# mjq11302010044/TPGSR

Measured on AMD Instinct MI355X. Metric: training img/s (16x64->32x128, bs=48/GPU), TPGSR-TSRN full train step, higher is better.
Workload: dtype bf16x2; 1 GPU; C3: TPGSR-TSRN = TSRN_TL (STN+mask) + CRNN teacher/student text prior, stu_iter 1, full train step (teacher fwd, student fwd+bwd, distill loss, prior dropout, SR fwd+bwd, ImageLoss(gradient), clip 0.25, Adam); tpg=crnn, batch_per_gpu=48, global_batch=48, parallelism=dp1, launch=recorded plans, plain launches: main + weight-gradient + teacher streams

## Files before the change

include/tpgsr_hip.h:

```cpp
#ifndef TPGSR_HIP_H
#define TPGSR_HIP_H

#ifdef __cplusplus
extern "C" {
#endif

#define TPGSR_ACT_NONE 0
#define TPGSR_ACT_RELU 1
#define TPGSR_ACT_MISH 2
#define TPGSR_ACT_TANH 3
#define TPGSR_ACT_PRELU 4

const char* tpgsr_last_error(void);
int tpgsr_version(void);
int tpgsr_sizeof(int which);

typedef struct {
  const float* in;
  const float* in2;
  const float* in_scale;
  const float* in_shift;
  const float* wt;
  const float* bias;
  float* out;
// ... 78 lines not shown
                       int layout, float* dw, float* db, int accumulate, float gscale ,
                       void* stream);

typedef struct tpgsr_wgrad_reduce_desc {
  const float* part;
  const float* dbpart;
  float* dw;
  float* db;
  int Z, K, Cin, Cout, KH, KW, layout, accumulate;
  float gscale;
  int blk0;
  int cin_ld;
  int reserved;
} tpgsr_wgrad_reduce_desc;
int tpgsr_wgrad_reduce_blocks2(int K, int Cin, int Cout, int KH, int KW, int layout, int cin_ld, int has_bias);
int tpgsr_wgrad_reduce_program(const tpgsr_wgrad_reduce_desc* descs_dev, int ndesc, int total_blocks, void* stream);

int tpgsr_pack_conv_weight(const float* w, int Cout, int Cin, int KH, int KW, int transposed, float wscale,
                           float* wt_f, float* wt_d, void* stream);
int tpgsr_pack_tail_weight(const float* w, int Co, int C, int KS, float* wt_f, float* wt_d, void* stream);

typedef struct {
  const float* src;
  float* dst_f;
  float* dst_d;
  int Cout, Cin, KH, KW;
  int kind, f_ld, f_coff;
  float wscale;
  int numel, blk0;
  const float* src2;
  const float* src3;
  int d_ld;
  int cin_ld;
} tpgsr_pack_desc;
typedef struct tpgsr_compose_bwd_desc {
  const float* dWc;
  const float* dbc;
  const float* W1;
  const float* b1;
  const float* wih0;
  const float* wih1;
  float* dW1;
  float* db1;
  float* dwih0;
  float* dwih1;
  float* dbih0;
  float* dbih1;
  int Cin, U, G, blk0;
} tpgsr_compose_bwd_desc;
int tpgsr_compose_bwd_blocks(int Cin, int U, int G);
int tpgsr_compose_bwd_program(const tpgsr_compose_bwd_desc* descs_dev, int ndesc, int total_blocks, void* stream);
int tpgsr_pack_blocks(int kind, int Cout, int Cin, int KH, int KW, long long numel);
int tpgsr_pack_program(const tpgsr_pack_desc* descs_dev, int ndesc, int total_blocks, void* stream);
typedef struct tpgsr_split_desc {
  const float* src;
  void* dst;
  int K, N, ld, kp, blk0;
  int cin;
} tpgsr_split_desc;
int tpgsr_split_bf_blocks(int K, int N);
int tpgsr_split_bf_program(const tpgsr_split_desc* descs_dev, int ndesc, int total_blocks, void* stream);
int tpgsr_bicubic_resize(const float* in_nchw, int N, int Ctot, int C, int H, int W, int OH, int OW, float scale, float shift,
                         float* out_nhwc, void* stream);
int tpgsr_aster_attention(const float* xproj, const float* sproj, const float* wv, const float* bv, const float* x, int N, int T, int A,
                          int D, float* alpha, float* context, void* stream);
int tpgsr_embed_concat(const int* ids, const float* emb, int V, int E, const float* ctx, int D, int N, float* out, void* stream);
int tpgsr_gru_cell(const float* gi, const float* gh, const float* h, int N, int Hd, float* hnew, void* stream);
int tpgsr_softmax_max(const float* logits, int N, int C, int* ids, float* score, int ld, int col, int* ids_next, void* stream);

void tpgsr_halo3_set_enabled(int on);
void tpgsr_wgrad3_set_enabled(int on);
void tpgsr_halo_set_colmajor_min_bytes(long long v);
void tpgsr_halo_set_min_taps(int v);
void tpgsr_halo_set_ne9(int on);
void tpgsr_panel_set_enabled(int on);
void tpgsr_panel_set_min_m(long long m);
void tpgsr_panel_set_k192(int on);
int tpgsr_halo_capacity(const tpgsr_conv_args* a);
int tpgsr_halo_trace(unsigned long long* buf);
int tpgsr_tr_probe(int* out, void* stream);
int tpgsr_mfma_bf16_probe(const void* a, const void* b, const float* c, float* d, int reps, void* stream);
int tpgsr_mfma_probe(float* out, int blocks, int iters, void* stream);
int tpgsr_copy(const float* src, float* dst, long long n, void* stream);
int tpgsr_zero(float* dst, long long n, void* stream);

// ... 230 lines not shown
```

tpgsr_amd/_lib.py:

```python
import ctypes as C
import os

import torch

_HERE = os.path.dirname(os.path.abspath(__file__))
LIB_PATH = os.path.join(_HERE, "libtpgsr_hip.so")

ACT_NONE, ACT_RELU, ACT_MISH, ACT_TANH, ACT_PRELU = 0, 1, 2, 3, 4
_ACT = {None: 0, "none": 0, "relu": 1, "mish": 2, "tanh": 3}

vp = C.c_void_p
ci = C.c_int
ll = C.c_longlong
cf = C.c_float


class ConvArgs(C.Structure):
    _fields_ = [("in_", vp), ("in2", vp), ("in_scale", vp), ("in_shift", vp), ("wt", vp), ("bias", vp), ("out", vp),
                ("bn_partial", vp),
                ("N", ci), ("H", ci), ("W", ci), ("Cin", ci),
                ("in_ld", ci), ("in_coff", ci), ("in2_ld", ci), ("in_act", ci), ("in_ps", ci),
                ("Cout", ci), ("KH", ci), ("KW", ci), ("pad_h", ci), ("pad_w", ci), ("OH", ci), ("OW", ci),
                ("out_ld", ci), ("out_coff", ci), ("out_act", ci), ("out_ps", ci),
                ("in_b", vp), ("cin_a", ci), ("in_b_ld", ci), ("in_dil_w", ci), ("wt_ld", ci), ("wt_coff", ci), ("stride_w", ci),
                ("terms", ci), ("kp", ci), ("wt_bf", vp), ("wt_bf_cin", ci), ("reserved0", ci),
                ("bnb_y", vp), ("bnb_mean", vp), ("bnb_rstd", vp), ("bnb_scale", vp), ("bnb_shift", vp), ("bnb_act", ci), ("bnb_store_dz", ci),
                ("fin_mode", ci), ("fin_accumulate", ci), ("fin_count", ll), ("fin_counter", vp), ("fin_gamma", vp), ("fin_beta", vp),
                ("fin_bias", vp), ("fin_scale", vp), ("fin_shift", vp), ("fin_mean", vp), ("fin_rstd", vp), ("fin_rm", vp), ("fin_rv", vp),
                ("fin_momentum", cf), ("fin_eps", cf), ("bn_row_tiles", ci), ("reserved1", ci), ("in2_scale", vp),
                ("sk_part", vp), ("sk_splits", ci), ("reserved2", ci)]


class WgradArgs(C.Structure):
    _fields_ = [("c", ConvArgs), ("dy", vp), ("dy_ld", ci), ("dy_coff", ci), ("dy_ps", ci), ("part", vp), ("dbpart", vp),
                ("zsplits", ci), ("reserved1", ci), ("dy_bf", vp)]


class GruWgradArgs(C.Structure):
    _fields_ = [("c", ConvArgs), ("dgi", vp), ("dghn", vp), ("h", vp), ("partC", vp), ("dbC", vp), ("partH", vp), ("dbH", vp),
                ("axis", ci), ("zsplits", ci)]


class BigruProjArgs(C.Structure):
    _fields_ = [("c", ConvArgs), ("w_hh", vp), ("b_hh", vp), ("h_out", vp), ("gates", vp), ("axis", ci), ("reserved", ci)]


class PackDesc(C.Structure):
    _fields_ = [("src", vp), ("dst_f", vp), ("dst_d", vp), ("Cout", ci), ("Cin", ci), ("KH", ci), ("KW", ci),
                ("kind", ci), ("f_ld", ci), ("f_coff", ci), ("wscale", cf), ("numel", ci), ("blk0", ci),
                ("src2", vp), ("src3", vp), ("d_ld", ci), ("cin_ld", ci)]


class ComposeBwdDesc(C.Structure):
    _fields_ = [("dWc", vp), ("dbc", vp), ("W1", vp), ("b1", vp), ("wih0", vp), ("wih1", vp), ("dW1", vp), ("db1", vp),
                ("dwih0", vp), ("dwih1", vp), ("dbih0", vp), ("dbih1", vp), ("Cin", ci), ("U", ci), ("G", ci), ("blk0", ci)]


class WgradReduceDesc(C.Structure):
    _fields_ = [("part", vp), ("dbpart", vp), ("dw", vp), ("db", vp), ("Z", ci), ("K", ci), ("Cin", ci), ("Cout", ci),
                ("KH", ci), ("KW", ci), ("layout", ci), ("accumulate", ci), ("gscale", cf), ("blk0", ci), ("cin_ld", ci),
                ("reserved", ci)]


class SplitDesc(C.Structure):
    _fields_ = [("src", vp), ("dst", vp), ("K", ci), ("N", ci), ("ld", ci), ("kp", ci), ("blk0", ci), ("cin", ci)]


class WgradBatchItem(C.Structure):
    _fields_ = [("w", WgradArgs), ("M", ci), ("K", ci), ("MB", ci), ("blk0", ci), ("nblk", ci), ("reserved0", ci), ("reserved1", ci), ("reserved2", ci)]


class ImageDesc(C.Structure):
    _fields_ = [("offset", ll), ("H", ci), ("W", ci), ("xb_off", ci), ("xk_off", ci), ("kx", ci), ("yb_off", ci), ("yk_off", ci), ("ky", ci)]


class BnDerive(C.Structure):
    _fields_ = [("rows", vp), ("nrows", ci), ("C", ci), ("count", ll), ("bias", vp), ("gamma", vp), ("beta", vp),
                ("running_mean", vp), ("running_var", vp), ("momentum", cf), ("eps", cf), ("scale", vp), ("shift", vp),
                ("save_mean", vp), ("save_rstd", vp), ("dgamma", vp), ("dbeta", vp), ("coef", vp), ("accumulate", ci), ("reserved", ci), ("flag", vp)]


class PlanArg(C.Union):
    _fields_ = [("p", vp), ("i", ll), ("f", C.c_double)]
# ... 7 lines not shown
    "tpgsr_plan_add_fork": (ci, [vp]),
    "tpgsr_plan_add_join": (ci, [vp]),
    "tpgsr_plan_set_arg": (ci, [vp, ci, ci, C.POINTER(PlanArg)]),
    "tpgsr_plan_run": (ci, [vp, vp, vp]),
    "tpgsr_plan_add_edge": (ci, [vp, ci, ci]),
    "tpgsr_plan_run3": (ci, [vp, vp, vp, vp]),
    "tpgsr_stream_create": (vp, [C.POINTER(C.c_uint), ci]),
    "tpgsr_plan_set_mode": (None, [ci, ci, C.c_ulonglong, ci]),
    "tpgsr_plan_get_mode": (ci, []),
    "tpgsr_plan_fuzz_point": (ci, [vp]),
    "tpgsr_spin": (ci, [ci, ci, cf, ci, vp]),
    "tpgsr_plan_set_stamp": (ci, [ci]),
    "tpgsr_plan_stamp_epoch": (ci, [vp]),
    "tpgsr_plan_read_stamps": (ci, [vp, C.POINTER(cf), C.POINTER(C.c_longlong), ci]),
    "tpgsr_stream_destroy": (ci, [vp]),
    "tpgsr_pack_program": (ci, [vp, ci, ci, vp]),
    "tpgsr_mfma_probe": (ci, [vp, ci, ci, vp]),
    "tpgsr_copy": (ci, [vp, vp, ll, vp]),
    "tpgsr_zero": (ci, [vp, ll, vp]),
    "tpgsr_version": (ci, []),
    "tpgsr_sizeof": (ci, [ci]),
    "tpgsr_conv_fwd": (ci, [C.POINTER(ConvArgs), vp]),
    "tpgsr_bigru_proj_supported": (ci, [C.POINTER(BigruProjArgs)]),
    "tpgsr_bigru_proj_fwd": (ci, [C.POINTER(BigruProjArgs), vp]),
    "tpgsr_bigru_proj_set_enabled": (None, [ci]),
    "tpgsr_affine_act_bnd": (ci, [C.POINTER(BnDerive), vp, ll, ci, vp, vp]),
    "tpgsr_affine_act_pool_bnd": (ci, [C.POINTER(BnDerive), vp, ci, ci, ci, ci, ci, ci, vp, vp]),
    "tpgsr_bn_bwd_apply_bnd": (ci, [C.POINTER(BnDerive), vp, vp, vp, ll, vp, vp, ci, vp, vp]),
    "tpgsr_wgrad_splits": (ci, [ci, ci, ci]),
    "tpgsr_conv_wgrad": (ci, [C.POINTER(WgradArgs), vp]),
    "tpgsr_wgrad_halo_plan": (ci, [C.POINTER(ConvArgs), C.POINTER(ci), C.POINTER(C.c_longlong)]),
    "tpgsr_wgrad_reduce": (ci, [vp, vp, ci, ci, ci, ci, ci, ci, ci, vp, vp, ci, cf, vp]),
    "tpgsr_pack_blocks": (ci, [ci, ci, ci, ci, ci, ll]),
    "tpgsr_conv_wgrad_batch_prepare": (ci, [C.POINTER(WgradArgs), C.POINTER(WgradBatchItem)]),
    "tpgsr_conv_wgrad_batch": (ci, [vp, ci, ci, ci, ci, vp]),
    "tpgsr_wgrad_reduce_blocks2": (ci, [ci, ci, ci, ci, ci, ci, ci, ci]),
    "tpgsr_wgrad_reduce_program": (ci, [vp, ci, ci, vp]),
    "tpgsr_compose_bwd_blocks": (ci, [ci, ci, ci]),
    "tpgsr_compose_bwd_program": (ci, [vp, ci, ci, vp]),
    "tpgsr_pack_conv_weight": (ci, [vp, ci, ci, ci, ci, ci, cf, vp, vp, vp]),
    "tpgsr_pack_tail_weight": (ci, [vp, ci, ci, ci, vp, vp, vp]),
    "tpgsr_bn_finalize": (ci, [vp, ci, ci, ll, vp, vp, vp, vp, vp, cf, cf, ci, vp, vp, vp, vp, vp]),
    "tpgsr_bn_stats": (ci, [vp, ll, ci, ci, vp, ci, vp]),
    "tpgsr_bn_bwd_reduce": (ci, [vp, vp, vp, ll, ci, vp, vp, vp, vp, ci, vp, ci, vp]),
    "tpgsr_bn_bwd_finalize": (ci, [vp, ci, ci, ll, vp, vp, vp, vp, vp, ci, vp, vp]),
    "tpgsr_bn_bwd_apply": (ci, [vp, vp, vp, ll, ci, vp, vp, ci, vp, vp, vp]),
    "tpgsr_affine_act": (ci, [vp, ll, ci, vp, vp, ci, vp, vp]),
    "tpgsr_affine_act_pool": (ci, [vp, ci, ci, ci, ci, vp, vp, ci, ci, ci, vp, vp]),
    "tpgsr_affine_act_pool_bwd": (ci, [vp, vp, ci, ci, ci, ci, vp, vp, ci, ci, ci, vp, vp]),
    "tpgsr_prelu_fwd": (ci, [vp, vp, ll, vp, vp]),
    "tpgsr_prelu_bwd": (ci, [vp, vp, vp, vp, ll, vp, vp, ci, vp]),
    "tpgsr_add": (ci, [vp, vp, ll, vp, vp]),
    "tpgsr_act_bwd": (ci, [vp, vp, ll, ci, vp, vp]),
    "tpgsr_nchw_to_nhwc": (ci, [vp, ci, ci, ci, ci, vp, vp]),
    "tpgsr_nhwc_to_nchw": (ci, [vp, ci, ci, ci, ci, vp, vp]),
    "tpgsr_reduce_partials": (ci, [vp, ci, ci, vp, ci, vp]),
    "tpgsr_bigru_fwd": (ci, [vp, vp, vp, ci, ci, ci, ci, vp, vp, vp]),
    "tpgsr_bigru_bwd": (ci, [vp, vp, vp, vp, vp, ci, ci, ci, ci, vp, vp, vp]),
    "tpgsr_bigru_bwd2": (ci, [vp, vp, vp, vp, vp, ci, ci, ci, ci, vp, vp, vp]),
    "tpgsr_gru_gate_math_probe": (ci, [vp, vp, vp, ci, vp]),
    "tpgsr_gru_wgrad_splits": (ci, [ll]),
    "tpgsr_gru_wgrad": (ci, [C.POINTER(GruWgradArgs), vp]),
    "tpgsr_tps_grid_fwd": (ci, [vp, vp, vp, ci, ci, ci, vp, vp, vp]),
    "tpgsr_tps_grid_bwd": (ci, [vp, vp, vp, vp, ci, ci, ci, vp, vp]),
    "tpgsr_grid_sample_fwd": (ci, [vp, vp, ci, ci, ci, ci, ci, ci, ci, vp, vp]),
    "tpgsr_grid_sample_bwd": (ci, [vp, vp, vp, ci, ci, ci, ci, ci, ci, ci, vp, vp, vp]),
# ... 127 lines not shown
```

tpgsr_amd/csrc/conv_mfma.hip:

```cpp
#include "common.h"
#include <stdlib.h>
#include <mutex>

#ifndef TPGSR_FRAG_PRELOAD
#define TPGSR_FRAG_PRELOAD 0
#endif
#include "conv_loader.h"

template <int LD, int SPLIT>
__global__ __launch_bounds__(256 * SPLIT) void conv_fwd_kernel(tpgsr_conv_args a, int M, int K, int vecB) {
  constexpr bool VEC_A = LD >= 0;
  __shared__ float As_[SPLIT][KC][ALD];
  __shared__ float Bs_[SPLIT][KC][BN];
  const int grp = SPLIT > 1 ? (int)(threadIdx.x >> 8) : 0;
  float (*As)[ALD] = As_[grp];
  float (*Bs)[BN] = Bs_[grp];
  const int tid = threadIdx.x & 255;
  const int lane = tid & 63, wave = tid >> 6;
  const int wm = wave & 1, wn = wave >> 1;
  const int nbn = (a.Cout + BN - 1) / BN;
  const int tile = xcd_remap(blockIdx.x, gridDim.x);
  const int mblk = tile / nbn;
  const int m0 = mblk * BM, n0 = (tile - mblk * nbn) * BN;
  const int nchunks_all = (K + KC - 1) / KC;
  const int nchunks = (nchunks_all + SPLIT - 1) / SPLIT;
  const int ch0 = grp * nchunks;

  const int aq = tid & 7;
  const int am0 = tid >> 3;
  PixelPos px0 = decode_pixel(a, m0 + am0, M);
  PixelPos px1 = decode_pixel(a, m0 + am0 + 32, M);
  const int bk0 = tid >> 4;
  const int bc = (tid & 15) * 4;

  float4 ra0, ra1, rb0, rb1;
  ARaw qa0, qa1;
  float4 qs = make_float4(1.f, 1.f, 1.f, 1.f), qt = make_float4(0.f, 0.f, 0.f, 0.f);
  constexpr int LDV = LD < 0 ? 0 : LD;
  const int Wr_ = real_w(a);
  const size_t in_floats = a.in_ps ? (size_t)a.N * a.H * a.W * a.Cin : (size_t)a.N * a.H * Wr_ * a.in_ld;
// ... 847 lines not shown
  if (idx >= total) return;
  int kw = idx % KS;
  size_t r = idx / KS;
  int kh = r % KS;
  r /= KS;
  int ci = r % C;
  int co = (int)(r / C);
  float v = w[idx];
  int NP = KS * Co;
  int np = kw * Co + co;
  if (wt_f) wt_f[((size_t)kh * C + ci) * NP + np] = v;
  if (wt_d) wt_d[((size_t)(KS - 1 - kh) * NP + np) * C + ci] = v;
}

extern "C" int tpgsr_pack_tail_weight(const float* w, int Co, int C, int KS, float* wt_f, float* wt_d, void* stream) {
  TPGSR_CHECK_ARG(w && (wt_f || wt_d), "tpgsr_pack_tail_weight: null pointer");
  size_t total = (size_t)Co * C * KS * KS;
  hipLaunchKernelGGL(pack_tail_weight_kernel, dim3(cdiv(total, 256)), dim3(256), 0, (hipStream_t)stream, w, Co, C, KS,
                     wt_f, wt_d);
  TPGSR_LAUNCH_CHECK("tpgsr_pack_tail_weight");
}

#define PK_TILED_MAX_TAPS 9
__host__ __device__ __forceinline__ bool pack_tiled(int kind, int Cout, int Cin, int KH, int KW) {
  return kind == 0 && KH * KW <= PK_TILED_MAX_TAPS && (long long)Cout * Cin >= 65536;
}
__host__ __device__ __forceinline__ int pack_desc_blocks(int kind, int Cout, int Cin, int KH, int KW, long long numel) {
  if (pack_tiled(kind, Cout, Cin, KH, KW)) return ((Cout + 31) / 32) * ((Cin + 31) / 32);
  return (int)((numel + 255) / 256);
}
extern "C" int tpgsr_pack_blocks(int kind, int Cout, int Cin, int KH, int KW, long long numel) {
  return pack_desc_blocks(kind, Cout, Cin, KH, KW, numel);
}

__global__ __launch_bounds__(256) void pack_program_kernel(const tpgsr_pack_desc* __restrict__ descs, int ndesc) {
  __shared__ int s_d;
  __shared__ float tile[32 * (32 * PK_TILED_MAX_TAPS + 1)];
  if (threadIdx.x == 0) {
    int lo = 0, hi = ndesc - 1;
    while (lo < hi) {
      int mid = (lo + hi + 1) >> 1;
      if (descs[mid].blk0 <= (int)blockIdx.x) lo = mid; else hi = mid - 1;
    }
    s_d = lo;
  }
  __syncthreads();
  const tpgsr_pack_desc d = descs[s_d];
  if (pack_tiled(d.kind, d.Cout, d.Cin, d.KH, d.KW)) {
    const int taps = d.KH * d.KW, R = 32 * taps, pitch = R | 1;
    const int nci = (d.Cin + 31) / 32;
    const int b = (int)blockIdx.x - d.blk0;
    const int co0 = (b / nci) * 32, ci0 = (b - (b / nci) * nci) * 32;
    const int cw = min(32, d.Cin - ci0) * taps;
    for (int e = threadIdx.x; e < 32 * R; e += 256) {
      const int row = e / R, pos = e - row * R;
      float v = 0.f;
      if (co0 + row < d.Cout && pos < cw) v = d.src[((size_t)(co0 + row) * d.Cin + ci0) * taps + pos] * d.wscale;
      tile[row * pitch + pos] = v;
    }
    __syncthreads();
    const int cin_ld = d.cin_ld > 0 ? d.cin_ld : d.Cin, d_ld = d.d_ld > 0 ? d.d_ld : d.Cin;
    if (d.dst_f) {
      for (int e = threadIdx.x; e < 32 * R; e += 256) {
        const int co_l = e & 31, rest = e >> 5;
        const int ci_l = rest & 31, tap = rest >> 5;
        if (co0 + co_l < d.Cout && ci0 + ci_l < d.Cin)
          d.dst_f[((size_t)tap * cin_ld + ci0 + ci_l) * d.f_ld + d.f_coff + co0 + co_l] = tile[co_l * pitch + ci_l * taps + tap];
      }
    }
    if (d.dst_d) {
      for (int e = threadIdx.x; e < 32 * R; e += 256) {
        const int ci_l = e & 31, rest = e >> 5;
        const int co_l = rest & 31, tap = rest >> 5;
        const int kh = tap / d.KW, kw = tap - kh * d.KW;
        if (co0 + co_l < d.Cout && ci0 + ci_l < d.Cin)
          d.dst_d[((size_t)((d.KH - 1 - kh) * d.KW + (d.KW - 1 - kw)) * d.Cout + co0 + co_l) * d_ld + ci0 + ci_l] = tile[co_l * pitch + ci_l * taps + tap];
      }
    }
    return;
  }
  long long idx = (long long)(blockIdx.x - d.blk0) * 256 + threadIdx.x;
  if (idx >= d.numel) return;
  if (d.kind == 5) {
    const int U = d.KH;
    const int g = (int)(idx / d.Cin), ci = (int)(idx - (long long)g * d.Cin);
    const float* wr = d.src + (size_t)g * U;
    float a0 = 0.f, a1 = 0.f, a2 = 0.f, a3 = 0.f;
    for (int u = 0; u < U; u += 4) {
      a0 = fmaf(wr[u], d.src2[(size_t)u * d.Cin + ci], a0);
      a1 = fmaf(wr[u + 1], d.src2[(size_t)(u + 1) * d.Cin + ci], a1);
      a2 = fmaf(wr[u + 2], d.src2[(size_t)(u + 2) * d.Cin + ci], a2);
      a3 = fmaf(wr[u + 3], d.src2[(size_t)(u + 3) * d.Cin + ci], a3);
    }
    const float v = (a0 + a1) + (a2 + a3);
    if (d.dst_f) d.dst_f[(size_t)ci * d.f_ld + d.f_coff + g] = v;
    if (d.dst_d) d.dst_d[(size_t)(d.f_coff + g) * d.Cin + ci] = v;
    return;
  }
  if (d.kind == 6) {
    const int U = d.KH, g = (int)idx;
    const float* wr = d.src + (size_t)g * U;
    float a0 = 0.f, a1 = 0.f;
    for (int u = 0; u < U; u += 2) {
      a0 = fmaf(wr[u], d.src2[u], a0);
      a1 = fmaf(wr[u + 1], d.src2[u + 1], a1);
    }
    d.dst_f[d.f_coff + g] = (a0 + a1) + d.src3[g];
    return;
  }
  float v = d.src[idx] * d.wscale;
  if (d.kind == 2) {
// ... 159 lines not shown
```

tpgsr_amd/engine.py:

```python
from __future__ import annotations

import contextlib
import ctypes as C
import math
import os
from typing import Dict, List, Optional

import torch

from . import kernels as K
from ._lib import PackDesc
from .kernels import ConvGeom, Plan, recording

F32 = torch.float32


class ParamArena:

    def __init__(self, module: torch.nn.Module):
        self.module = module
        self.flat: Optional[torch.Tensor] = None
        self.grad: Optional[torch.Tensor] = None
        self.offsets: Dict[str, int] = {}
        self.numel = 0
# ... 488 lines not shown
        from ._lib import ComposeBwdDesc, load
        lib = load()
        arr = (ComposeBwdDesc * len(items))()
        blk, keep = 0, []
        for d, (L, dWc, dbc) in zip(arr, items):
            P, G, gp = self.P, self.G, L.gp
            t = dict(dWc=dWc, dbc=dbc, W1=P[L.w1name], b1=P[L.b1name], wih0=P[gp + "weight_ih_l0"], wih1=P[gp + "weight_ih_l0_reverse"],
                     dW1=G[L.w1name], db1=G[L.b1name], dwih0=G[gp + "weight_ih_l0"], dwih1=G[gp + "weight_ih_l0_reverse"],
                     dbih0=G[gp + "bias_ih_l0"], dbih1=G[gp + "bias_ih_l0_reverse"])
            for k, v in t.items():
                setattr(d, k, v.data_ptr())
            keep += list(t.values())
            d.Cin, d.U, d.G, d.blk0 = L.Cin, L.U, 96, blk
            blk += lib.tpgsr_compose_bwd_blocks(L.Cin, L.U, 96)
        table = torch.frombuffer(bytearray(bytes(arr)), dtype=torch.uint8).to(self.device)
        if K._REC is not None:
            K._REC.keep += keep
        with K.side():
            K.compose_bwd_program(table, len(items), blk)

    def add_pack(self, src, dst_f, dst_d, Cout=0, Cin=0, KH=1, KW=1, kind=0, f_ld=0, f_coff=0, wscale=1.0, src2=None, src3=None,
                 numel=None, d_ld=0, cin_ld=0):
        self._pack.append((src, dst_f, dst_d, Cout, Cin, KH, KW, kind, f_ld, f_coff, wscale, src2, src3, numel, d_ld, cin_ld,
                           getattr(self, "_pack_group", 0)))

    def register_operand(self, *tensors, cins=None):
        for i, t in enumerate(tensors):
            if t is not None:
                assert t.dim() == 2 and t.is_contiguous()
                self._operands.append(t)
                t._tpgsr_cin = K.block_order_cin(t.shape[0], cins[i] if cins else 0)
                t._tpgsr_group = getattr(self, "_pack_group", 0)

    def _finish_split_table(self):
        from ._lib import SplitDesc, load
        self._split_tabs = {}
        self._split_n = 0
        ops, seen = [], set()
        for t in self._operands:
            if t.data_ptr() not in seen:
                seen.add(t.data_ptr())
                ops.append(t)
        if K.POLICY == "f32" or not ops:
            return
        lib = load()
        self._split_keep = []
        for grp in sorted({getattr(t, "_tpgsr_group", 0) for t in ops}):
            sel = [t for t in ops if getattr(t, "_tpgsr_group", 0) == grp]
            arr = (SplitDesc * len(sel))()
            blk = 0
            for d, t in zip(arr, sel):
                Kd, N = t.shape
                kp = (Kd + 31) // 32 * 32
                twin = torch.zeros(3 * ((N + 31) // 32 * 32) * kp, dtype=torch.bfloat16, device=self.device)
                cin = getattr(t, "_tpgsr_cin", 0)
                K.register_bf_twin(t, twin, kp, cin)
                d.src, d.dst, d.K, d.N, d.ld, d.kp, d.blk0, d.cin = t.data_ptr(), twin.data_ptr(), Kd, N, N, kp, blk, cin
                blk += lib.tpgsr_split_bf_blocks(Kd, N)
                self._split_keep += [t, twin]
            self._split_tabs[grp] = (torch.frombuffer(bytearray(bytes(arr)), dtype=torch.uint8).to(self.device), len(sel), blk)
        self._split_n = len(ops)

    def _finish_pack_table(self):
        from ._lib import load
        lib = load()
        self._pack_tabs = {}
        self._pack_keep = []
        for grp in sorted({e[16] for e in self._pack}):
            sel = [e for e in self._pack if e[16] == grp]
            arr = (PackDesc * len(sel))()
            blk = 0
            for d, (src, dst_f, dst_d, Cout, Cin, KH, KW, kind, f_ld, f_coff, wscale, src2, src3, numel, d_ld, cin_ld, _g) in zip(arr, sel):
                d.src, d.dst_f = src.data_ptr(), dst_f.data_ptr()
                d.dst_d = dst_d.data_ptr() if dst_d is not None else None
                d.src2 = src2.data_ptr() if src2 is not None else None
                d.src3 = src3.data_ptr() if src3 is not None else None
                d.Cout, d.Cin, d.KH, d.KW, d.kind, d.f_ld, d.f_coff, d.wscale = Cout, Cin, KH, KW, kind, f_ld, f_coff, wscale
                d.d_ld, d.cin_ld = d_ld, cin_ld
                cnt = src.numel() if numel is None else numel
                d.numel, d.blk0 = cnt, blk
                blk += lib.tpgsr_pack_blocks(kind, Cout, Cin, KH, KW, cnt)
                self._pack_keep += [src, dst_f, dst_d, src2, src3]
            self._pack_tabs[grp] = (torch.frombuffer(bytearray(bytes(arr)), dtype=torch.uint8).to(self.device), len(sel), blk)

    def pack_group(self, grp):
        if grp in self._pack_tabs:
            K.pack_program(*self._pack_tabs[grp])
        if grp in self._split_tabs:
            K.split_bf_program(*self._split_tabs[grp])

    def pack_all(self):
        for grp in sorted(set(self._pack_tabs) | set(self._split_tabs)):
            self.pack_group(grp)

    def _param_key(self):
        return (sum(p._version for p in self.P.values()), self._kernel_writes, self.arena.flat.data_ptr(), bool(getattr(self, "_split_tabs", None)))

    @staticmethod
    def _plan_splits(plan) -> bool:
        v = getattr(plan, "_tpgsr_splits", None)
        if v is None:
            v = any(op[0] == "tpgsr_split_bf_program" for op in plan.ops)
            try:
                plan._tpgsr_splits = v
            except AttributeError:
                pass
        return v

    def pack_if_stale(self, pack_plan):
        capturing = (not K.DRYRUN) and torch.cuda.is_current_stream_capturing()
        key = self._param_key()
        check = (not K.DRYRUN) and (not capturing) and os.environ.get("TPGSR_PACK_CHECK") == "1"
        splits = self._plan_splits(pack_plan)
        if capturing or key != self._packed_key or (splits and not self._packed_split) or os.environ.get("TPGSR_PACK_ALWAYS") == "1":
            pack_plan.run()
            self._packed_key = None if capturing else key
            self._packed_split = splits
            if check:
                self._packed_sum = self._arena_checksum()
        elif check and getattr(self, "_packed_sum", None) is not None and self._arena_checksum() != self._packed_sum:
            raise RuntimeError(f"{type(self.module).__name__}: the parameters changed behind torch's version counters since the operands were "
                               "packed (a write through p.data / a raw pointer / a flat arena view?) -- call module._engine().invalidate_packed() "
                               "after such writes (TPGSR_PACK_CHECK=1 found this)")

    def _arena_checksum(self):
        w = self.arena.flat.view(torch.int32).to(torch.int64)
        return (int(w.sum().item()), int((w * w).sum().item()))

    def invalidate_packed(self):
        self._kernel_writes += 1
        self._packed_key = None

    def note_packed(self):
        self._packed_key = self._param_key()
        self._packed_split = bool(K.CONV_TERMS)

    def bind(self, device):
        rebuilt = self.arena.ensure(device)
        if not rebuilt and self.device == device:
            return
        self.device = device
        self._plans.clear()
        self._packed_key = None
        self._scratch.clear()
        self._live.clear()
        self._pack = []
        self._operands = []
        self._bn_layers = []
        m = self.module
        self.P = dict(m.named_parameters())
        self.B = dict(m.named_buffers())
        self.G = {}
        for name, p in self.P.items():
            o = self.arena.offsets[name]
            self.G[name] = self.arena.grad[o:o + p.numel()]
        for name, b in self.B.items():
            if b.device != device:
                raise RuntimeError(f"buffer {name} is on {b.device}, parameters on {device}: call module.to(device) first")
        self._build_layers()
        self._finish_pack_table()
        self._finish_split_table()

    def flush_counters(self):
        if self._pending_batches and self.device is not None:
            for n, b in self.B.items():
                if n.endswith("num_batches_tracked"):
                    b += self._pending_batches
        self._pending_batches = 0

    def _two_pass(self, key, record):
        if key not in self._plans:
            if K.POLICY != "f32" and self._operands and not self._split_tabs:
                self._finish_split_table()
            ws = _Ws(self.device)
            record(ws, False)
            self._plans[key] = record(ws, True)
        return self._plans[key]


class TSRNEngine(_EngineBase):

    STN_POOLS = [(2, 2), (2, 2), (2, 2), (2, 2), (1, 2), (1, 1)]

    def __init__(self, module: torch.nn.Module, grid_align_corners: bool = False):
        super().__init__(module)
        self.grid_align_corners = grid_align_corners
        self.overlap_wgrad = os.environ.get("TPGSR_OVERLAP_WGRAD", "1") != "0"
        self.defer_reduce = os.environ.get("TPGSR_DEFER_REDUCE", "1") != "0"
        self.leaf_stn = os.environ.get("TPGSR_LEAF_STN", "1") != "0"
        self.leaf_early = os.environ.get("TPGSR_LEAF_EARLY", "0") == "1"
        self.leaf_strip = os.environ.get("TPGSR_LEAF_STRIP", "1") != "0"
        self.split_leaf_reduce = os.environ.get("TPGSR_SPLIT_LEAF_REDUCE", "1") != "0"
        self.side_batch_blocks = max(1, int(os.environ.get("TPGSR_SIDE_BATCH_BLOCKS", "2")))
        self.side_batch_tail = os.environ.get("TPGSR_SIDE_BATCH_TAIL", "1") != "0"

    def _build_layers(self):
        m = self.module
        self.in_planes = m.in_planes
        self.srb = m.srb_nums
        self.stn = bool(m.stn)
        self.C = self.P["block1.0.weight"].shape[0]
        self.block1 = ConvLayer(self, "block1.0.weight", "block1.0.bias", 9, 9, 4, 4, need_dgrad=False)
        self.block1_dx = FoldedDgrad(self, "block1.0.weight") if self.stn else None
        self.tl = hasattr(m, "infoGen")
        self.rrb = []
        for i in range(self.srb):
# ... 442 lines not shown
```

tpgsr_amd/engine_crnn.py:

```python
from __future__ import annotations

import os
from typing import Optional

import torch

from . import kernels as K
from .engine import BNLayer, ConvLayer, F32, _EngineBase
from .kernels import ConvGeom, Plan, recording


class Conv0Im2col:

    def __init__(self, eng, wname, bname):
        self.eng, self.wname, self.bname = eng, wname, bname
        self.w, self.b = eng.P[wname], eng.P[bname]
        assert tuple(self.w.shape[1:]) == (1, 3, 3)
        self.Cout, self.Cin = self.w.shape[0], 12
        dev = eng.device
        self.wt_f = torch.zeros(12, self.Cout, dtype=F32, device=dev)
        self.wt_d = torch.zeros(self.Cout, 12, dtype=F32, device=dev)
        eng.add_pack(self.w, self.wt_f, self.wt_d, Cout=self.Cout, Cin=9, KH=1, KW=1, kind=0, f_ld=self.Cout, d_ld=12)
        eng.register_operand(self.wt_f, self.wt_d)

# ... 35 lines not shown

    def wgrad(self, N, H, W, x, dy_p):
        eng, g = self.eng, ConvGeom(N, H, W, self.Cin, self.Cout)
        Z = K.wgrad_splits(g.M, g.K, g.Cout)
        part, dbp = eng.wgrad_buffers(Z * g.K * g.Cout, Z * g.Cout)
        with K.side():
            K.conv_wgrad(K.make_wgrad_args(K.make_conv_args(g, x), dy_p, part, dbp, dy_ld=self.Cp))
            K.wgrad_reduce(part, dbp, Z, g, eng.G[self.wname], eng.G[self.bname], accumulate=True)


class LstmLayer:

    def __init__(self, eng, prefix: str):
        self.eng, self.prefix = eng, prefix
        P, dev = eng.P, eng.device
        r = prefix + ".rnn."
        self.r = r
        self.Hh = Hh = P[r + "weight_hh_l0"].shape[1]
        self.Cin = Cin = P[r + "weight_ih_l0"].shape[1]
        G4 = 4 * Hh
        self.wih_f = torch.empty(Cin, 2 * G4, dtype=F32, device=dev)
        self.wih_d = torch.empty(2 * G4, Cin, dtype=F32, device=dev)
        self.bih = torch.empty(2 * G4, dtype=F32, device=dev)
        self.bhh = torch.empty(2, G4, dtype=F32, device=dev)
        self.whh_f = torch.empty(2, Hh, G4, dtype=F32, device=dev)
        for d, suf in enumerate(("", "_reverse")):
            eng.add_pack(P[r + "weight_ih_l0" + suf], self.wih_f, self.wih_d[d * G4:(d + 1) * G4], Cout=G4, Cin=Cin, kind=0,
                         f_ld=2 * G4, f_coff=d * G4)
            eng.add_pack(P[r + "bias_ih_l0" + suf], self.bih[d * G4:(d + 1) * G4], None, kind=2)
            eng.add_pack(P[r + "bias_hh_l0" + suf], self.bhh[d], None, kind=2)
            eng.add_pack(P[r + "weight_hh_l0" + suf], self.whh_f[d], None, Cout=G4, Cin=Hh, kind=0, f_ld=G4)
        eng.register_operand(self.wih_f, self.wih_d)
        nout = P[prefix + ".embedding.weight"].shape[0]
        self.emb = (ConvLayer if nout % 4 == 0 else PaddedLinear)(eng, prefix + ".embedding.weight", prefix + ".embedding.bias")

    def fwd(self, N, T, x, G, gh, Cst, out, e, **loader):
        Hh, G4, P = self.Hh, 4 * self.Hh, self.eng.P
        K.conv_fwd(K.make_conv_args(ConvGeom(N, 1, T, self.Cin, 2 * G4), x, self.wih_f, G, bias=self.bih, **loader))
        if K.LSTM_SEQ and Hh == 256 and N <= 64 and K.lstm_seq_coresident(self.eng.device):
            if not hasattr(self, "_seq"):
                self._seq = {}
            gran = K.LSTM_GRANULE and T <= 31
            key = (K.current_stream().cuda_stream, gran, N)
            if key not in self._seq:
                self._seq[key] = K.lstm_seq_granule_buffers(self.eng.device) if gran else K.lstm_seq_buffers(self.eng.device)
            hx, sync = self._seq[key]
            (K.lstm_seq_fwdg if gran else K.lstm_seq_fwd)(G, self.whh_f, self.bhh, Cst, out, hx, sync, N, T, Hh)
            self.emb.fwd(N, 1, T, out, e)
            return
        S = Hh // (32 * K.LSTM_FWD_KCHUNKS)
        for s in range(T):
            if s > 0:
                a = [out.data_ptr() + 4 * ((s - 1 if d == 0 else T - s) * 2 * Hh + d * Hh) for d in range(2)]
                K.lstm_rec_gemm(a[0], a[1], T * 2 * Hh, self.whh_f[0], self.whh_f[1], N, Hh, G4, S, gh)
            K.lstm_step_fwd(G, gh if s > 0 else None, S, self.bhh, Cst, out, N, T, Hh, s)
        self.emb.fwd(N, 1, T, out, e)

    def bwd(self, N, T, x, G, Cst, out, de, dout, dhc, dcc, dx, dx_bnb=None, **loader):
        eng, P, Gd, r = self.eng, self.eng.P, self.eng.G, self.r
        Hh, G4 = self.Hh, 4 * self.Hh
        batch = K.LSTM_WGRAD_BATCH and K.CONV_TERMS > 0 and K.deferring() and isinstance(self.emb, (ConvLayer, PaddedLinear))
        if not batch:
            self.emb.wgrad(N, 1, T, out, de)
        self.emb.dgrad(N, 1, T, de, dout)
        S = G4 // (32 * K.LSTM_BWD_KCHUNKS)
        seq = K.LSTM_SEQ_BWD and Hh == 256 and N <= 64 and K.lstm_seq_coresident(self.eng.device)
        if seq:
# ... 300 lines not shown
```

Before: 8821 img/s.

## Fuse bf16 triple-split twin writes into the tiled weight pack kernel

The tiled weight-pack kernel now also writes the three-way bf16 split twins (MFMA tiled layout) directly from its shared-memory tile, for operands whose every pack entry qualifies. Those operands are dropped from the separate split_bf program. This removes a per-step read and rewrite of packed f32 weights. The cost is more complex descriptor planning and eligibility checks, with a risk of layout mismatch on edge cases. The CRNN PaddedLinear embedding is also forced into pack group 0.

```diff
diff --git a/include/tpgsr_hip.h b/include/tpgsr_hip.h
--- a/include/tpgsr_hip.h
+++ b/include/tpgsr_hip.h
@@ -134,6 +134,10 @@
   const float* src3;
   int d_ld;
   int cin_ld;
+  void* bf_f;
+  void* bf_d;
+  int bf_f_kp, bf_f_nb32, bf_f_cin, bf_f_koff;
+  int bf_d_kp, bf_d_nb32, bf_d_cin, bf_d_koff;
 } tpgsr_pack_desc;
 typedef struct tpgsr_compose_bwd_desc {
   const float* dWc;
@@ -153,6 +157,7 @@
 int tpgsr_compose_bwd_blocks(int Cin, int U, int G);
 int tpgsr_compose_bwd_program(const tpgsr_compose_bwd_desc* descs_dev, int ndesc, int total_blocks, void* stream);
 int tpgsr_pack_blocks(int kind, int Cout, int Cin, int KH, int KW, long long numel);
+int tpgsr_pack_tiled(int kind, int Cout, int Cin, int KH, int KW);
 int tpgsr_pack_program(const tpgsr_pack_desc* descs_dev, int ndesc, int total_blocks, void* stream);
 typedef struct tpgsr_split_desc {
   const float* src;
diff --git a/tpgsr_amd/_lib.py b/tpgsr_amd/_lib.py
--- a/tpgsr_amd/_lib.py
+++ b/tpgsr_amd/_lib.py
@@ -48,7 +48,9 @@
 class PackDesc(C.Structure):
     _fields_ = [("src", vp), ("dst_f", vp), ("dst_d", vp), ("Cout", ci), ("Cin", ci), ("KH", ci), ("KW", ci),
                 ("kind", ci), ("f_ld", ci), ("f_coff", ci), ("wscale", cf), ("numel", ci), ("blk0", ci),
-                ("src2", vp), ("src3", vp), ("d_ld", ci), ("cin_ld", ci)]
+                ("src2", vp), ("src3", vp), ("d_ld", ci), ("cin_ld", ci), ("bf_f", vp), ("bf_d", vp),
+                ("bf_f_kp", ci), ("bf_f_nb32", ci), ("bf_f_cin", ci), ("bf_f_koff", ci),
+                ("bf_d_kp", ci), ("bf_d_nb32", ci), ("bf_d_cin", ci), ("bf_d_koff", ci)]
 
 
 class ComposeBwdDesc(C.Structure):
@@ -122,6 +124,7 @@
     "tpgsr_wgrad_halo_plan": (ci, [C.POINTER(ConvArgs), C.POINTER(ci), C.POINTER(C.c_longlong)]),
     "tpgsr_wgrad_reduce": (ci, [vp, vp, ci, ci, ci, ci, ci, ci, ci, vp, vp, ci, cf, vp]),
     "tpgsr_pack_blocks": (ci, [ci, ci, ci, ci, ci, ll]),
+    "tpgsr_pack_tiled": (ci, [ci, ci, ci, ci, ci]),
     "tpgsr_conv_wgrad_batch_prepare": (ci, [C.POINTER(WgradArgs), C.POINTER(WgradBatchItem)]),
     "tpgsr_conv_wgrad_batch": (ci, [vp, ci, ci, ci, ci, vp]),
     "tpgsr_wgrad_reduce_blocks2": (ci, [ci, ci, ci, ci, ci, ci, ci, ci]),
diff --git a/tpgsr_amd/csrc/conv_mfma.hip b/tpgsr_amd/csrc/conv_mfma.hip
--- a/tpgsr_amd/csrc/conv_mfma.hip
+++ b/tpgsr_amd/csrc/conv_mfma.hip
@@ -6,6 +6,7 @@
 #define TPGSR_FRAG_PRELOAD 0
 #endif
 #include "conv_loader.h"
+#include "conv_xbf_common.h"
 
 template <int LD, int SPLIT>
 __global__ __launch_bounds__(256 * SPLIT) void conv_fwd_kernel(tpgsr_conv_args a, int M, int K, int vecB) {
@@ -919,6 +920,7 @@
 extern "C" int tpgsr_pack_blocks(int kind, int Cout, int Cin, int KH, int KW, long long numel) {
   return pack_desc_blocks(kind, Cout, Cin, KH, KW, numel);
 }
+extern "C" int tpgsr_pack_tiled(int kind, int Cout, int Cin, int KH, int KW) { return pack_tiled(kind, Cout, Cin, KH, KW) ? 1 : 0; }
 
 __global__ __launch_bounds__(256) void pack_program_kernel(const tpgsr_pack_desc* __restrict__ descs, int ndesc) {
   __shared__ int s_d;
@@ -964,6 +966,54 @@
           d.dst_d[((size_t)((d.KH - 1 - kh) * d.KW + (d.KW - 1 - kw)) * d.Cout + co0 + co_l) * d_ld + ci0 + ci_l] = tile[co_l * pitch + ci_l * taps + tap];
       }
     }
+    if (d.bf_f) {
+      const int KB16 = d.bf_f_kp >> 4;
+      const size_t plane = (size_t)d.bf_f_nb32 * KB16 * 512;
+      unsigned short* dst = reinterpret_cast<unsigned short*>(d.bf_f);
+      for (int e = threadIdx.x; e < 128 * taps; e += 256) {
+        const int co_l = e & 31, g = (e >> 5) & 3, tap = e >> 7;
+        const int cig = ci0 + g * 8;
+        const int k = d.bf_f_cin > 0 ? ((ci0 >> 5) * taps + tap) * 32 + g * 8 : d.bf_f_koff + tap * cin_ld + cig;
+        if (co0 + co_l >= d.Cout || cig >= cin_ld || k >= d.bf_f_kp) continue;
+        __bf16 h[8][3];
+#pragma unroll
+        for (int j = 0; j < 8; ++j) split_bf<3>(tile[co_l * pitch + (g * 8 + j) * taps + tap], h[j]);
+        const int nn = d.f_coff + co0 + co_l;
+        const size_t off = ((((size_t)(nn >> 5) * KB16 + (k >> 4)) * 64) + ((k >> 3) & 1) * 32 + (nn & 31)) * 8;
+#pragma unroll
+        for (int t = 0; t < 3; ++t) {
+          bf16x8 v;
+#pragma unroll
+          for (int j = 0; j < 8; ++j) v[j] = h[j][t];
+          *reinterpret_cast<bf16x8*>(dst + t * plane + off) = v;
+        }
+      }
+    }
+    if (d.bf_d) {
+      const int KB16 = d.bf_d_kp >> 4;
+      const size_t plane = (size_t)d.bf_d_nb32 * KB16 * 512;
+      unsigned short* dst = reinterpret_cast<unsigned short*>(d.bf_d);
+      for (int e = threadIdx.x; e < 128 * taps; e += 256) {
+        const int ci_l = e & 31, g = (e >> 5) & 3, tap = e >> 7;
+        const int kh = tap / d.KW, kw = tap - kh * d.KW;
+        const int tf = (d.KH - 1 - kh) * d.KW + (d.KW - 1 - kw);
+        const int cog = co0 + g * 8;
+        const int k = d.bf_d_cin > 0 ? ((co0 >> 5) * taps + tf) * 32 + g * 8 : d.bf_d_koff + tf * d.Cout + cog;
+        if (ci0 + ci_l >= d.Cin || cog >= d.Cout || k >= d.bf_d_kp) continue;
+        __bf16 h[8][3];
+#pragma unroll
+        for (int j = 0; j < 8; ++j) split_bf<3>(tile[(g * 8 + j) * pitch + ci_l * taps + tap], h[j]);
+        const int nn = ci0 + ci_l;
+        const size_t off = ((((size_t)(nn >> 5) * KB16 + (k >> 4)) * 64) + ((k >> 3) & 1) * 32 + (nn & 31)) * 8;
+#pragma unroll
+        for (int t = 0; t < 3; ++t) {
+          bf16x8 v;
+#pragma unroll
+          for (int j = 0; j < 8; ++j) v[j] = h[j][t];
+          *reinterpret_cast<bf16x8*>(dst + t * plane + off) = v;
+        }
+      }
+    }
     return;
   }
   long long idx = (long long)(blockIdx.x - d.blk0) * 256 + threadIdx.x;
diff --git a/tpgsr_amd/engine.py b/tpgsr_amd/engine.py
--- a/tpgsr_amd/engine.py
+++ b/tpgsr_amd/engine.py
@@ -544,69 +544,130 @@
                 t._tpgsr_cin = K.block_order_cin(t.shape[0], cins[i] if cins else 0)
                 t._tpgsr_group = getattr(self, "_pack_group", 0)
 
+    def _make_twins(self):
+        self._twins = False
+        self._split_ops, seen = [], set()
+        for t in self._operands:
+            if t.data_ptr() not in seen:
+                seen.add(t.data_ptr())
+                self._split_ops.append(t)
+        if K.POLICY == "f32" or not self._split_ops:
+            return
+        self._split_keep = []
+        for t in self._split_ops:
+            Kd, N = t.shape
+            kp = (Kd + 31) // 32 * 32
+            twin = torch.zeros(3 * ((N + 31) // 32 * 32) * kp, dtype=torch.bfloat16, device=self.device)
+            K.register_bf_twin(t, twin, kp, getattr(t, "_tpgsr_cin", 0))
+            self._split_keep += [t, twin]
+        self._twins = True
+
+    def _plane_target(self, e, lib):
+        src, dst_f, dst_d, Cout, Cin, KH, KW, kind, f_ld, f_coff, wscale, src2, src3, numel, d_ld, cin_ld, _g = e
+        tiled = self._twins and bool(lib.tpgsr_pack_tiled(kind, Cout, Cin, KH, KW))
+        taps, out = KH * KW, []
+        for side, dst in (("f", dst_f), ("d", dst_d)):
+            if dst is None:
+                continue
+            hit = None
+            for t in self._split_ops:
+                o = dst.data_ptr() - t.data_ptr()
+                if 0 <= o < t.numel() * 4:
+                    hit = (t,) + divmod(o // 4, t.shape[1])
+                    break
+            if hit is None:
+                continue
+            t, row, col = hit
+            tw, fields = getattr(t, "_tpgsr_twin", None), None
+            if tiled and tw is not None and col == 0:
+                kp, cin_t = tw[1], tw[2]
+                ch, ld, own = (cin_ld or Cin, f_ld, Cin) if side == "f" else (Cout, d_ld or Cin, Cout)
+                ok = ld == t.shape[1] and (f_coff % 32 == 0 if side == "f" else True)
+                if cin_t > 0:
+                    ok = ok and cin_t == own == ch and row == 0 and t.shape[0] == taps * ch
+                else:
+                    ok = ok and ch % 8 == 0 and row % 8 == 0
+                if ok:
+                    fields = (tw[0], kp, (t.shape[1] + 31) // 32, cin_t, row)
+            out.append((side, t, fields))
+        return out
+
+    def _finish_pack_table(self):
+        from ._lib import load
+        lib = load()
+        self._pack_tabs = {}
+        self._pack_keep = []
+        self._pack_planes = set()
+        targets = [self._plane_target(e, lib) for e in self._pack]
+        whole = {}
+        for tg in targets:
+            for side, t, fields in tg:
+                whole[t.data_ptr()] = whole.get(t.data_ptr(), True) and fields is not None
+        self._plane_ops = {p for p, ok in whole.items() if ok}
+        for grp in sorted({e[16] for e in self._pack}):
+            sel = [(e, tg) for e, tg in zip(self._pack, targets) if e[16] == grp]
+            arr = (PackDesc * len(sel))()
+            blk = 0
+            for d, ((src, dst_f, dst_d, Cout, Cin, KH, KW, kind, f_ld, f_coff, wscale, src2, src3, numel, d_ld, cin_ld, _g), tg) in zip(arr, sel):
+                d.src, d.dst_f = src.data_ptr(), dst_f.data_ptr()
+                d.dst_d = dst_d.data_ptr() if dst_d is not None else None
+                d.src2 = src2.data_ptr() if src2 is not None else None
+                d.src3 = src3.data_ptr() if src3 is not None else None
+                d.Cout, d.Cin, d.KH, d.KW, d.kind, d.f_ld, d.f_coff, d.wscale = Cout, Cin, KH, KW, kind, f_ld, f_coff, wscale
+                d.d_ld, d.cin_ld = d_ld, cin_ld
+                for side, t, fields in tg:
+                    if t.data_ptr() in self._plane_ops:
+                        twin, kp, nb32, cin_t, row = fields
+                        if side == "f":
+                            d.bf_f, d.bf_f_kp, d.bf_f_nb32, d.bf_f_cin, d.bf_f_koff = twin.data_ptr(), kp, nb32, cin_t, row
+                        else:
+                            d.bf_d, d.bf_d_kp, d.bf_d_nb32, d.bf_d_cin, d.bf_d_koff = twin.data_ptr(), kp, nb32, cin_t, row
+                        self._pack_planes.add(grp)
+                cnt = src.numel() if numel is None else numel
+                d.numel, d.blk0 = cnt, blk
+                blk += lib.tpgsr_pack_blocks(kind, Cout, Cin, KH, KW, cnt)
+                self._pack_keep += [src, dst_f, dst_d, src2, src3]
+            self._pack_tabs[grp] = (torch.frombuffer(bytearray(bytes(arr)), dtype=torch.uint8).to(self.device), len(sel), blk)
+
     def _finish_split_table(self):
         from ._lib import SplitDesc, load
         self._split_tabs = {}
         self._split_n = 0
-        ops, seen = [], set()
-        for t in self._operands:
-            if t.data_ptr() not in seen:
-                seen.add(t.data_ptr())
-                ops.append(t)
-        if K.POLICY == "f32" or not ops:
+        if not self._twins:
             return
         lib = load()
-        self._split_keep = []
+        ops = [t for t in self._split_ops if t.data_ptr() not in self._plane_ops]
         for grp in sorted({getattr(t, "_tpgsr_group", 0) for t in ops}):
             sel = [t for t in ops if getattr(t, "_tpgsr_group", 0) == grp]
             arr = (SplitDesc * len(sel))()
             blk = 0
             for d, t in zip(arr, sel):
                 Kd, N = t.shape
-                kp = (Kd + 31) // 32 * 32
-                twin = torch.zeros(3 * ((N + 31) // 32 * 32) * kp, dtype=torch.bfloat16, device=self.device)
-                cin = getattr(t, "_tpgsr_cin", 0)
-                K.register_bf_twin(t, twin, kp, cin)
+                twin, kp, cin = t._tpgsr_twin
                 d.src, d.dst, d.K, d.N, d.ld, d.kp, d.blk0, d.cin = t.data_ptr(), twin.data_ptr(), Kd, N, N, kp, blk, cin
                 blk += lib.tpgsr_split_bf_blocks(Kd, N)
-                self._split_keep += [t, twin]
             self._split_tabs[grp] = (torch.frombuffer(bytearray(bytes(arr)), dtype=torch.uint8).to(self.device), len(sel), blk)
-        self._split_n = len(ops)
-
-    def _finish_pack_table(self):
-        from ._lib import load
-        lib = load()
-        self._pack_tabs = {}
-        self._pack_keep = []
-        for grp in sorted({e[16] for e in self._pack}):
-            sel = [e for e in self._pack if e[16] == grp]
-            arr = (PackDesc * len(sel))()
-            blk = 0
-            for d, (src, dst_f, dst_d, Cout, Cin, KH, KW, kind, f_ld, f_coff, wscale, src2, src3, numel, d_ld, cin_ld, _g) in zip(arr, sel):
-                d.src, d.dst_f = src.data_ptr(), dst_f.data_ptr()
-                d.dst_d = dst_d.data_ptr() if dst_d is not None else None
-                d.src2 = src2.data_ptr() if src2 is not None else None
-                d.src3 = src3.data_ptr() if src3 is not None else None
-                d.Cout, d.Cin, d.KH, d.KW, d.kind, d.f_ld, d.f_coff, d.wscale = Cout, Cin, KH, KW, kind, f_ld, f_coff, wscale
-                d.d_ld, d.cin_ld = d_ld, cin_ld
-                cnt = src.numel() if numel is None else numel
-                d.numel, d.blk0 = cnt, blk
-                blk += lib.tpgsr_pack_blocks(kind, Cout, Cin, KH, KW, cnt)
-                self._pack_keep += [src, dst_f, dst_d, src2, src3]
-            self._pack_tabs[grp] = (torch.frombuffer(bytearray(bytes(arr)), dtype=torch.uint8).to(self.device), len(sel), blk)
+        self._split_n = len(self._split_ops)
+
+    def _finish_tables(self):
+        self._make_twins()
+        self._finish_pack_table()
+        self._finish_split_table()
 
     def pack_group(self, grp):
         if grp in self._pack_tabs:
             K.pack_program(*self._pack_tabs[grp])
         if grp in self._split_tabs:
             K.split_bf_program(*self._split_tabs[grp])
+        if K._REC is not None and self._twins:
+            K._REC._tpgsr_splits = True
 
     def pack_all(self):
         for grp in sorted(set(self._pack_tabs) | set(self._split_tabs)):
             self.pack_group(grp)
 
     def _param_key(self):
-        return (sum(p._version for p in self.P.values()), self._kernel_writes, self.arena.flat.data_ptr(), bool(getattr(self, "_split_tabs", None)))
+        return (sum(p._version for p in self.P.values()), self._kernel_writes, self.arena.flat.data_ptr(), bool(getattr(self, "_twins", False)))
 
     @staticmethod
     def _plan_splits(plan) -> bool:
@@ -670,8 +731,7 @@
             if b.device != device:
                 raise RuntimeError(f"buffer {name} is on {b.device}, parameters on {device}: call module.to(device) first")
         self._build_layers()
-        self._finish_pack_table()
-        self._finish_split_table()
+        self._finish_tables()
 
     def flush_counters(self):
         if self._pending_batches and self.device is not None:
@@ -682,8 +742,8 @@
 
     def _two_pass(self, key, record):
         if key not in self._plans:
-            if K.POLICY != "f32" and self._operands and not self._split_tabs:
-                self._finish_split_table()
+            if K.POLICY != "f32" and self._operands and not self._twins:
+                self._finish_tables()
             ws = _Ws(self.device)
             record(ws, False)
             self._plans[key] = record(ws, True)
diff --git a/tpgsr_amd/engine_crnn.py b/tpgsr_amd/engine_crnn.py
--- a/tpgsr_amd/engine_crnn.py
+++ b/tpgsr_amd/engine_crnn.py
@@ -91,7 +91,12 @@
             eng.add_pack(P[r + "weight_hh_l0" + suf], self.whh_f[d], None, Cout=G4, Cin=Hh, kind=0, f_ld=G4)
         eng.register_operand(self.wih_f, self.wih_d)
         nout = P[prefix + ".embedding.weight"].shape[0]
-        self.emb = (ConvLayer if nout % 4 == 0 else PaddedLinear)(eng, prefix + ".embedding.weight", prefix + ".embedding.bias")
+        if nout % 4 == 0:
+            self.emb = ConvLayer(eng, prefix + ".embedding.weight", prefix + ".embedding.bias")
+        else:
+            grp, eng._pack_group = getattr(eng, "_pack_group", 0), 0
+            self.emb = PaddedLinear(eng, prefix + ".embedding.weight", prefix + ".embedding.bias")
+            eng._pack_group = grp
 
     def fwd(self, N, T, x, G, gh, Cst, out, e, **loader):
         Hh, G4, P = self.Hh, 4 * self.Hh, self.eng.P
```

After: 8835 img/s, median of 6. About the same (+0.2%).
